# Shinzef/BlenderRayTracer

Measured on AMD Instinct MI355X. Metric: Msamples/s (pixels×spp/s) at 1/2/4/8 MI355X; % HBM roofline; RMS vs JS ref, higher is better.
Workload: dtype f64; 1 GPU; config3_rtow_1920x1080_512spp; scene=rtow.json, width=1920, height=1080, spp=512, max_depth=5, primitives=486, accel=auto, parallelism=1 GPU

## Files before the change

### __graft_entry__.py

```python
import os
import sys

ROOT = os.path.dirname(os.path.abspath(__file__))
if ROOT not in sys.path:
    sys.path.insert(0, ROOT)


def build() -> None:
    from blenderraytracer_amd import build as b
    b.build_lib(force=True)
    b.build_cli(force=True)
    b.build_napi(force=True)
    from oracle import binding
    binding.build()
    sys.path.insert(0, os.path.join(ROOT, "tests"))
    import hostcheck_binding
    hostcheck_binding.build()
    hostcheck_binding.lib(("RT_HOST_COUNTERS=1",))
    counting = ("RT_HOST_COUNTERS=1", "RT_TRI_FILTER=1")
    hostcheck_binding.lib(counting)
    hostcheck_binding.lib(counting + ("RT_TRI_EXIT=0",))
    hostcheck_binding.lib(("RT_HOST_COUNTERS=1", "RT_TRI_EXIT=0"))
    import texcheck_binding
    texcheck_binding.build()
    import lightcheck_binding
    lightcheck_binding.build()
    import guidedcheck_binding
    guidedcheck_binding.build()
    import neecheck_binding
    for mutation in (0, 1, 2):
        neecheck_binding.build(mutation)
    import filterxcheck_binding
    filterxcheck_binding.build()
    import errcheck_binding
    errcheck_binding.build()
    import vguidedcheck_binding
    vguidedcheck_binding.build()
    import blenderraytracer_amd
    from blenderraytracer_amd import capi
    capi.load_library()


def smoke() -> None:
    import numpy as np

    from blenderraytracer_amd import capi
    from blenderraytracer_amd.renderer import GpuRayTracer
    from blenderraytracer_amd.scene import load_scene_json
    from oracle import binding

    rt = GpuRayTracer(64, 48, seed=7, device=0, precision=capi.RT_PREC_F64)
    assert rt.load_from_json(load_scene_json("sample_scene.json"))
    rt.update_render_settings({"maxBounces": 4, "samples": 4})
    r = rt.render(want=("mean", "segments"))
    o = binding.render(rt.packed(), rt.settings())
    assert np.array_equal(r["segments"], o["segments"]), "segment counts differ from the oracle"
    err = np.max(np.abs(r["mean"] - o["mean"]))
    assert err <= 1e-12, f"GPU vs oracle max abs diff {err}"
    assert np.array_equal(r["rgba8"], o["rgba8"])
    print(f"smoke ok: 64x48x4spp sample_scene, {rt.last_stats.kernel_ms:.3f} ms kernel, max|diff| {err:.1e}")
    rt.close()
    rt = GpuRayTracer(48, 27, seed=7, device=0, precision=capi.RT_PREC_F64)
    assert rt.load_from_json(load_scene_json("rtow.json"))
    rt.update_render_settings({"maxBounces": 5, "samples": 4})
    lib = capi.load_library()
    assert lib.rt_scene_walk(rt.scene_handle(), capi.RT_PREC_F64, capi.RT_ACCEL_AUTO) == 2, "RTOW should walk the grid"
    r = rt.render(want=("mean", "segments"))
    o = binding.render(rt.packed(), rt.settings())
    assert np.array_equal(r["segments"], o["segments"]), "RTOW segment counts differ from the oracle"
    err = np.max(np.abs(r["mean"] - o["mean"]))
    assert err <= 1e-12, f"RTOW GPU vs oracle max abs diff {err}"
    assert np.array_equal(r["rgba8"], o["rgba8"])
    print(f"smoke ok: 48x27x4spp RTOW (grid walk), max|diff| {err:.1e}")
    rt.close()


if __name__ == "__main__":
    build()
    if len(sys.argv) > 1 and sys.argv[1] == "smoke":
        smoke()
```

### blenderraytracer_amd/build.py

```python
import hashlib
import json
import os
import shutil
import subprocess
import sys

HERE = os.path.dirname(os.path.abspath(__file__))
CSRC = os.path.join(HERE, "csrc")
LIBDIR = os.path.join(HERE, "lib")
REPO = os.path.dirname(HERE)
ARCH = os.environ.get("RT_OFFLOAD_ARCH", "gfx950")
HIPCC = os.environ.get("HIPCC", shutil.which("hipcc") or "/opt/rocm/bin/hipcc")

SOURCES = ["pt_trace.hip", "pt_onewave.hip", "pt_guided.hip", "pt_error.hip", "rt_capi.cpp", "scene_json.cpp"]
SOURCE_FLAGS = {"pt_onewave.hip": ["-mllvm", "-amdgpu-use-amdgpu-trackers=1"]}
HIP_FLAGS = ["-O3", "-std=c++17", f"--offload-arch={ARCH}", "-ffp-contract=off", "-fPIC",
             "-mllvm", "-structurizecfg-skip-uniform-regions=1",
             "-Wall", "-Wno-unused-function", "-I", os.path.join(REPO, "include")]


def _run(cmd):
    print(" ".join(cmd), flush=True)
    subprocess.check_call(cmd)

# ... 14 lines not shown
            if os.path.isfile(p):
                h.update(f.encode())
                with open(p, "rb") as fh:
                    h.update(fh.read())
    return h.hexdigest()[:16]


def _git(*args):
    try:
        return subprocess.run(["git", "-C", REPO, *args], capture_output=True, text=True, timeout=10).stdout.strip()
    except Exception:
        return ""


def write_build_info():
    info = {"commit": _git("rev-parse", "--short", "HEAD") or None,
            "sources_modified": bool(_git("status", "--porcelain", "--", CSRC, os.path.join(REPO, "include"),
                                          os.path.abspath(__file__))),
            "source_digest": source_digest()}
    with open(os.path.join(LIBDIR, "build_info.json"), "w") as f:
        json.dump(info, f)
    return info


def read_build_info():
    try:
        with open(os.path.join(LIBDIR, "build_info.json")) as f:
            return json.load(f)
    except (OSError, ValueError):
        return None


def build_lib(force=False):
    os.makedirs(LIBDIR, exist_ok=True)
    target = os.path.join(LIBDIR, "librt_hip.so")
    deps = [os.path.join(CSRC, f) for f in os.listdir(CSRC)] + [os.path.join(REPO, "include", f) for f in os.listdir(os.path.join(REPO, "include"))]
    if not force and not _stale(target, deps):
        return target
    objs, procs = [], []
    for src in SOURCES:
        obj = os.path.join(LIBDIR, os.path.splitext(src)[0] + ".o")
        cmd = [HIPCC, *HIP_FLAGS, *SOURCE_FLAGS.get(src, []), "-c", os.path.join(CSRC, src), "-o", obj]
        print(" ".join(cmd), flush=True)
        procs.append((cmd, subprocess.Popen(cmd)))
        objs.append(obj)
    failed = [cmd for cmd, p in procs if p.wait() != 0]
    if failed:
        raise subprocess.CalledProcessError(1, failed[0])
    _run([HIPCC, "-shared", f"--offload-arch={ARCH}", "-o", target, *objs])
    write_build_info()
    return target


def build_napi(force=False):
    node_inc = os.environ.get("NODE_INCLUDE", "/usr/include/node")
    if not os.path.exists(os.path.join(node_inc, "node_api.h")):
        print("node_api.h not found: skipping the N-API addon")
        return None
    target = os.path.join(LIBDIR, "rt_napi.node")
    src = os.path.join(CSRC, "napi_addon.cpp")
    if not os.path.exists(src):
        return None
    if not force and not _stale(target, [src, os.path.join(REPO, "include", "rt_hip.h"), os.path.join(LIBDIR, "librt_hip.so")]):
        return target
    _run(["g++", "-O2", "-std=c++17", "-fPIC", "-shared", "-I", node_inc, "-I", os.path.join(REPO, "include"),
          src, "-o", target, "-L", LIBDIR, "-lrt_hip", "-Wl,-rpath,$ORIGIN"])
    return target


def build_cli(force=False):
    target = os.path.join(LIBDIR, "rt_render_cli")
    src = os.path.join(CSRC, "rt_cli.cpp")
    deps = [src, os.path.join(LIBDIR, "librt_hip.so")] + [os.path.join(REPO, "include", f)
                                                          for f in os.listdir(os.path.join(REPO, "include"))]
    if not force and not _stale(target, deps):
        return target
    _run(["g++", "-O2", "-std=c++17", "-Wall", "-I", os.path.join(REPO, "include"), src, "-o", target,
          "-L", LIBDIR, "-lrt_hip", "-Wl,-rpath,$ORIGIN", "-Wl,-rpath-link,/opt/rocm/lib"])
    return target


def main(argv=None):
    argv = sys.argv[1:] if argv is None else argv
    force = "--force" in argv
    print(build_lib(force))
    print(build_cli(force))
    if "--napi" in argv:
        print(build_napi(force))


if __name__ == "__main__":
    main()
```

### blenderraytracer_amd/csrc/kernel_select.h

```cpp
#pragma once
#include <algorithm>
#include <cstdlib>
#include <cstring>
#include <type_traits>

#include "pt_core.h"

namespace rt {

#ifndef RT_MIN_WAVES_PER_SIMD
#define RT_MIN_WAVES_PER_SIMD 6
#endif
#ifndef RT_BVH_WAVES_PER_SIMD
#define RT_BVH_WAVES_PER_SIMD 4
#endif
#ifndef RT_BVH_WAVES_F32
#define RT_BVH_WAVES_F32 5
#endif

#ifndef RT_SPHERES_WAVES_PER_SIMD
#define RT_SPHERES_WAVES_PER_SIMD 5
#endif
#ifndef RT_SPHERES_WAVES_F32
#define RT_SPHERES_WAVES_F32 6
// ... 10 lines not shown
#define RT_GRID_WAVES_PER_SIMD 5
#endif
#ifndef RT_GRID_WAVES_F32
#define RT_GRID_WAVES_F32 6
#endif

template <class R, int ACC>
constexpr int waves_per_simd() {
    if constexpr (ACC == ACC_GRID || ACC == ACC_GRID_LDS || ACC == ACC_GRID_LDS_LEAN)
        return sizeof(R) == 8 ? RT_GRID_WAVES_PER_SIMD : RT_GRID_WAVES_F32;
    if constexpr (ACC == ACC_BVH_SPHERES) return sizeof(R) == 8 ? RT_SPHERES_WAVES_PER_SIMD : RT_SPHERES_WAVES_F32;
    if constexpr (ACC == ACC_BVH_SPHERES_LDS) return sizeof(R) == 8 ? RT_LDS_OCC_F64 : RT_LDS_OCC_F32;
    if constexpr (ACC == ACC_BVH_TRI_LDS) return sizeof(R) == 8 ? RT_BVH_WAVES_PER_SIMD : RT_BVH_WAVES_F32;
    return walk_of<ACC>() >= ACC_BVH ? (sizeof(R) == 8 ? RT_BVH_WAVES_PER_SIMD : RT_BVH_WAVES_F32) : RT_MIN_WAVES_PER_SIMD;
}

#ifndef RT_LDS_WAVES_F64
#define RT_LDS_WAVES_F64 8
#endif
#ifndef RT_LDS_WAVES_F32
#define RT_LDS_WAVES_F32 12
#endif
#ifndef RT_GRID_LDS_WAVES_F64
#define RT_GRID_LDS_WAVES_F64 4
#endif
#ifndef RT_GRID_LDS_WAVES_F32
#define RT_GRID_LDS_WAVES_F32 12
#endif
#ifndef RT_TRI_LDS_WAVES_F64
#define RT_TRI_LDS_WAVES_F64 16
#endif
#ifndef RT_TRI_LDS_WAVES_F32
#define RT_TRI_LDS_WAVES_F32 4
#endif
template <class R, int ACC = ACC_BVH_SPHERES_LDS>
constexpr int lds_waves() {
    if constexpr (ACC == ACC_GRID_LDS || ACC == ACC_GRID_LDS_LEAN) return sizeof(R) == 8 ? RT_GRID_LDS_WAVES_F64 : RT_GRID_LDS_WAVES_F32;
    if constexpr (ACC == ACC_BVH_TRI_LDS) return sizeof(R) == 8 ? RT_TRI_LDS_WAVES_F64 : RT_TRI_LDS_WAVES_F32;
    return sizeof(R) == 8 ? RT_LDS_WAVES_F64 : RT_LDS_WAVES_F32;
}

struct WideLds {
    int n, entries;
    RT_HD int boxes() const { return 0; }
    RT_HD int kids() const { return 48 * n; }
    RT_HD int stacks() const { return 56 * n; }
    RT_HD size_t bytes(int waves) const { return (size_t)56 * n + (size_t)waves * entries * 64 * 4; }
};
template <class R, int ACC>
constexpr long long lds_budget(int fewer_workgroups = 0) {
    return 160 * 1024 / (4 * waves_per_simd<R, ACC>() / lds_waves<R, ACC>() - fewer_workgroups);
}
template <class R, int ACC>
constexpr long long lds_fixed_bytes() { return (long long)lds_waves<R, ACC>() * 3 * 64 * 8 + 256; }

#ifndef RT_LDS_NODES
#define RT_LDS_NODES 1
#endif
#ifndef RT_LDS_GRID
#define RT_LDS_GRID 1
#endif
#ifndef RT_MAT_LDS
#define RT_MAT_LDS 0
#endif
#ifndef RT_LDS_TRI
#define RT_LDS_TRI 0
#endif
#ifndef RT_LEAN
#define RT_LEAN 1
#endif
constexpr int kWalkTree = -2;
inline int parse_bvh_walk(const char* e) {
    return e && !strncmp(e, "skip", 4) ? ACC_BVH : e && !strncmp(e, "two", 3) ? ACC_BVH_STACK
         : e && !strncmp(e, "grid", 4) ? ACC_GRID : e && !strncmp(e, "tree", 4) ? kWalkTree : ACC_BVH_SPHERES;
}
struct SelectKnobs {
    int bvh_walk = ACC_BVH_SPHERES;
    int lean = RT_LEAN;
    int lds_grid = RT_LDS_GRID;
    int lds_nodes = RT_LDS_NODES;
    int lds_tri = RT_LDS_TRI;
    int tri_lds_nodes = RT_TRI_TOP_NODES;
};
inline int env_int(const char* name, int def) {
    const char* e = getenv(name);
    return e ? atoi(e) : def;
}
inline SelectKnobs knobs_from_env() {
    SelectKnobs k;
    k.bvh_walk = parse_bvh_walk(getenv("RT_BVH_WALK"));
    k.lean = env_int("RT_LEAN", RT_LEAN);
    k.lds_grid = env_int("RT_LDS_GRID", RT_LDS_GRID);
    k.lds_nodes = env_int("RT_LDS_NODES", RT_LDS_NODES);
    k.lds_tri = env_int("RT_LDS_TRI", RT_LDS_TRI);
    k.tri_lds_nodes = std::max(0, std::min(env_int("RT_TRI_LDS_NODES", RT_TRI_TOP_NODES), RT_TRI_TOP_NODES));
    return k;
}

struct SceneFacts {
    int num_lights, num_tex, num_tri_nodes, num_tri_wide, num_sphere_wide, num_grid_cells, use_grid, num_planes,
        num_boxes, background, cam_ortho, stack_entries, num_mats;
    size_t grid_lds_bytes;
    int num_emitters;
};
template <class R>
SceneFacts scene_facts(const SceneView<R>& sc) {
    return SceneFacts{sc.num_lights, sc.num_tex, sc.num_tri_nodes, sc.num_tri_wide, sc.num_sphere_wide, sc.num_grid_cells,
                      sc.use_grid, sc.num_planes, sc.num_boxes, sc.background, sc.cam_ortho, sc.stack_entries,
                      sc.num_mats, grid_lds_bytes(sc), sc.num_emitters};
}

constexpr int kAccelCount = ACC_BVH_STACK_NEE + 1;
constexpr bool lds_form(int acc) {
    return acc == ACC_BVH_SPHERES_LDS || acc == ACC_GRID_LDS || acc == ACC_GRID_LDS_LEAN || acc == ACC_BVH_TRI_LDS;
}
constexpr int plain_of(int acc) {
    return acc == ACC_GRID_LDS_LEAN ? ACC_GRID_LDS : acc == ACC_BVH_STACK_LEAN ? ACC_BVH_STACK
         : acc == ACC_BRUTE_LEAN ? ACC_BRUTE : acc;
}
constexpr int walk_report(int acc) {
    return acc == ACC_BRUTE || acc == ACC_BRUTE_LEAN || acc == ACC_BRUTE_TEX || acc == ACC_BRUTE_LIT || acc == ACC_BRUTE_NEE ? 0
         : acc == ACC_GRID || acc == ACC_GRID_LDS || acc == ACC_GRID_LDS_LEAN ? 2 : 1;
}

struct KernelChoice {
    Accel acc;
    bool lds;
    size_t lds_bytes;
    int tri_lds_nodes;
};

template <int A = 0, class F>
auto with_acc(int acc, F&& f) -> decltype(f(std::integral_constant<int, 0>{})) {
    if constexpr (A + 1 == kAccelCount) return f(std::integral_constant<int, A>{});
    else return acc == A ? f(std::integral_constant<int, A>{}) : with_acc<A + 1>(acc, f);
}

template <class R>
KernelChoice select_kernel(const SceneFacts& s, int aa_mode, bool bvh, bool pool, const SelectKnobs& k) {
    const auto one_wave = [](Accel acc) { return KernelChoice{acc, false, 0, 0}; };
    if (s.num_emitters > 0) return one_wave(bvh ? ACC_BVH_STACK_NEE : ACC_BRUTE_NEE);
    if (s.num_lights > 0) return one_wave(bvh ? ACC_BVH_STACK_LIT : ACC_BRUTE_LIT);
    if (s.num_tex > 0) return one_wave(bvh ? ACC_BVH_STACK_TEX : ACC_BRUTE_TEX);
    const auto lean = [&](int feat) {
        if (k.lean == 0 || (k.lean == 2 && feat != 0)) return false;
        return (s.num_planes == 0 || (feat & F_PLANES)) && (s.num_boxes == 0 || (feat & F_BOXES)) &&
               (s.num_tri_nodes == 0 || (feat & F_TRIS)) && s.background == 0 && !s.cam_ortho && aa_mode == 0;
    };
    Accel walk = ACC_BRUTE;
    if (bvh && s.num_tri_nodes > 0) walk = k.bvh_walk == ACC_BVH ? ACC_BVH : ACC_BVH_STACK;
    else if (bvh && s.num_grid_cells > 0 && (k.bvh_walk == ACC_GRID || (k.bvh_walk == ACC_BVH_SPHERES && s.use_grid)))
        walk = ACC_GRID;
    else if (bvh) walk = k.bvh_walk == ACC_BVH || k.bvh_walk == ACC_BVH_STACK ? (Accel)k.bvh_walk : ACC_BVH_SPHERES;
    if (!pool) return one_wave(walk);
    const int entries = std::min(s.stack_entries, RT_BVH_STACK);
    if (walk == ACC_BRUTE && lean(feat_of<ACC_BRUTE_LEAN>())) return one_wave(ACC_BRUTE_LEAN);
    if (walk == ACC_GRID && k.lds_grid >= 1) {
        const size_t b = ((s.grid_lds_bytes + 15) & ~(size_t)15) + (RT_MAT_LDS ? sizeof(MatRec<R>) * (size_t)s.num_mats : 0);
        if ((long long)b + lds_fixed_bytes<R, ACC_GRID_LDS>() <= lds_budget<R, ACC_GRID_LDS>(RT_MAT_LDS ? 1 : 0))
            return KernelChoice{lean(feat_of<ACC_GRID_LDS_LEAN>()) ? ACC_GRID_LDS_LEAN : ACC_GRID_LDS, true, b, 0};
    }
    if (walk == ACC_BVH_SPHERES && k.lds_nodes >= (sizeof(R) == 8 ? 2 : 1) && s.num_sphere_wide > 0) {
        constexpr int W = lds_waves<R, ACC_BVH_SPHERES_LDS>();
        const size_t b = WideLds{s.num_sphere_wide, entries}.bytes(W);
        if ((long long)b + lds_fixed_bytes<R, ACC_BVH_SPHERES_LDS>() <= lds_budget<R, ACC_BVH_SPHERES_LDS>())
            return KernelChoice{ACC_BVH_SPHERES_LDS, true, b, 0};
    }
    if (walk == ACC_BVH_STACK) {
        if (k.lds_tri >= (sizeof(R) == 8 ? 1 : 2) && s.num_tri_wide > 0) {
            constexpr int W = lds_waves<R, ACC_BVH_TRI_LDS>();
            const long long fixed = (long long)W * entries * 64 * 4 + lds_fixed_bytes<R, ACC_BVH_TRI_LDS>();
            const long long n = std::min<long long>({(long long)s.num_tri_wide, (long long)k.tri_lds_nodes,
                                                     (lds_budget<R, ACC_BVH_TRI_LDS>() - fixed) / 56});
            if (n >= 64) return KernelChoice{ACC_BVH_TRI_LDS, true, WideLds{(int)n, entries}.bytes(W), (int)n};
        }
        if (lean(feat_of<ACC_BVH_STACK_LEAN>())) return one_wave(ACC_BVH_STACK_LEAN);
    }
    return one_wave(walk);
}

}
```

### blenderraytracer_amd/csrc/pt_core.h

```cpp
#pragma once
#include <hip/hip_runtime.h>
#include <math.h>
#include <stdint.h>
#include <string.h>
#include "js_math.h"

#define RT_HD __host__ __device__ __forceinline__
#ifndef RT_COLD_BG
#define RT_COLD_BG 1
#endif
#if RT_COLD_BG && defined(__HIP_DEVICE_COMPILE__)
#define RT_COLD __attribute__((noinline))
#else
#define RT_COLD
#endif
#define RT_COLD_HD __host__ __device__ RT_COLD

namespace rt {

template <class R> RT_HD R js_pow(R x, R y) {
    if constexpr (sizeof(R) == 8) return jsm::pow(x, y);
    else return pow(x, y);
}
template <class R> RT_HD R js_exp(R x) {
// ... 1234 lines not shown
    if ((e = fabs(p.y - b.mny)) < best) { best = e; n = mk<R>(0, -1, 0); }
    if ((e = fabs(p.y - b.mxy)) < best) { best = e; n = mk<R>(0, 1, 0); }
    if ((e = fabs(p.z - b.mnz)) < best) { best = e; n = mk<R>(0, 0, -1); }
    if ((e = fabs(p.z - b.mxz)) < best) { best = e; n = mk<R>(0, 0, 1); }
    return n;
}

template <class R, int FEAT = F_ALL>
RT_HD Hit<R> hit_record(const SceneView<R>& sc, V3<R> o, V3<R> d, const Closest<R>& c) {
    Hit<R> h;
    h.p = o + d * c.t;
    h.mat = c.mat;
    if ((FEAT & (F_PLANES | F_BOXES | F_TRIS)) == 0 || c.kind == HIT_SPHERE) {
        const SphereRec<R> s = sc.spheres[c.idx];
#if RT_DIV_RCP
        set_face(h, d, vdiv_rcp(h.p - mk(s.cx, s.cy, s.cz), sc.sphere_r[c.idx], sc.sphere_inv_r[c.idx]));
#else
        set_face(h, d, vdiv(h.p - mk(s.cx, s.cy, s.cz), sc.sphere_r[c.idx]));
#endif
    } else if ((FEAT & F_PLANES) != 0 && c.kind == HIT_PLANE) {
        const PlaneRec<R> p = sc.planes[c.idx];
        set_face(h, d, mk(p.nx, p.ny, p.nz));
    } else if ((FEAT & F_BOXES) != 0 && c.kind == HIT_BOX) {
        const BoxRec<R> b = sc.boxes[c.idx];
        const R eps = (R)1e-6;
        V3<R> n;
        if (fabs(h.p.x - b.mnx) < eps) n = mk<R>(-1, 0, 0);
        else if (fabs(h.p.x - b.mxx) < eps) n = mk<R>(1, 0, 0);
        else if (fabs(h.p.y - b.mny) < eps) n = mk<R>(0, -1, 0);
        else if (fabs(h.p.y - b.mxy) < eps) n = mk<R>(0, 1, 0);
        else if (fabs(h.p.z - b.mnz) < eps) n = mk<R>(0, 0, -1);
        else if (sizeof(R) == 8 || fabs(h.p.z - b.mxz) < eps) n = mk<R>(0, 0, 1);
        else n = box_nearest_face(h.p, b);
        set_face(h, d, n);
    } else {
        const TriRec<R> tr = sc.tris[c.idx];
        set_face(h, d, mk(tr.nx, tr.ny, tr.nz));
    }
    return h;
}

template <class R>
RT_HD V3<R> random_in_unit_sphere(Rng<R>& g) {
    int64_t x, y, z;
    do {
        RT_HCOUNT(HC_SPHERE_DRAW_ROUNDS, 1);
        x = (int64_t)g.next_u24() - (1 << 23);
        y = (int64_t)g.next_u24() - (1 << 23);
        z = (int64_t)g.next_u24() - (1 << 23);
    } while (x * x + y * y + z * z >= ((int64_t)1 << 46));
    return mk((R)x * (R)0x1p-23, (R)y * (R)0x1p-23, (R)z * (R)0x1p-23);
}

template <class R>
RT_HD V3<R> random_in_unit_disk(Rng<R>& g) {
    int64_t x, y;
    do {
        RT_HCOUNT(HC_DISK_DRAW_ROUNDS, 1);
        x = (int64_t)g.next_u24() - (1 << 23);
        y = (int64_t)g.next_u24() - (1 << 23);
    } while (x * x + y * y >= ((int64_t)1 << 46));
    return mk<R>((R)x * (R)0x1p-23, (R)y * (R)0x1p-23, 0);
}

template <class R> RT_HD R fade(R t) { return t * t * t * (t * (t * (R)6 - (R)15) + (R)10); }
template <class R> RT_HD R lerp(R t, R a, R b) { return a + t * (b - a); }
template <class R> RT_HD R grad(int hash, R x, R y, R z) {
    int h = hash & 15;
    R u = h < 8 ? x : y;
    R v = h < 4 ? y : (h == 12 || h == 14) ? x : z;
    return ((h & 1) == 0 ? u : -u) + ((h & 2) == 0 ? v : -v);
}
template <class R>
__host__ __device__ R perlin(const int* p, R x, R y, R z) {
    R fx0 = floor(x), fy0 = floor(y), fz0 = floor(z);
    int X = ((int)(long long)fx0) & 255, Y = ((int)(long long)fy0) & 255, Z = ((int)(long long)fz0) & 255;
    R fx = x - fx0, fy = y - fy0, fz = z - fz0;
    R u = fade(fx), v = fade(fy), w = fade(fz);
    int A = p[X] + Y, AA = p[A] + Z, AB = p[A + 1] + Z;
    int B = p[X + 1] + Y, BA = p[B] + Z, BB = p[B + 1] + Z;
    return lerp(w,
                lerp(v, lerp(u, grad(p[AA], fx, fy, fz), grad(p[BA], fx - (R)1, fy, fz)),
                     lerp(u, grad(p[AB], fx, fy - (R)1, fz), grad(p[BB], fx - (R)1, fy - (R)1, fz))),
                lerp(v, lerp(u, grad(p[AA + 1], fx, fy, fz - (R)1), grad(p[BA + 1], fx - (R)1, fy, fz - (R)1)),
                     lerp(u, grad(p[AB + 1], fx, fy - (R)1, fz - (R)1), grad(p[BB + 1], fx - (R)1, fy - (R)1, fz - (R)1))));
}


template <class R>
__host__ __device__ RT_COLD V3<R> background_hdri(const SceneView<R>& sc, V3<R> d) {
    const R I = sc.sky_intensity;
    V3<R> dir = normalize(d);
    V3<R> sun = normalize(mk<R>(-0.3, 0.6, -0.5));
    R sd = js_max<R>(0, dot(dir, sun));
    R mask = sd > ((R)1 - (R)0.04) ? (R)1 : (R)0;
    V3<R> sun_c = mk<R>(1.0, 0.95, 0.8) * (mask * (R)20);
    R corona = js_max<R>(0, (sd - ((R)1 - (R)0.2)) / (R)0.2);
    V3<R> cor_c = mk<R>(1.0, 0.8, 0.6) * (js_pow<R>(corona, (R)2) * (R)3);
    R y = dir.y;
    V3<R> sky_c = mk<R>(0.3, 0.5, 0.8) * (js_max<R>(0, y * (R)0.5 + (R)0.5) * (R)2);
    V3<R> gnd_c = mk<R>(0.2, 0.15, 0.1) * js_max<R>(0, -y * (R)0.3);
    V3<R> sc_c = mk<R>(0.8, 0.9, 1.0) * (js_pow<R>(js_max<R>(0, (R)1 - fabs(y)), (R)2) * (R)0.3);
    return ((((sky_c + gnd_c) + sc_c) + sun_c) + cor_c) * I;
}

template <class R>
// ... 150 lines not shown
```

### blenderraytracer_amd/csrc/pt_path.h

```cpp
#pragma once
#include <type_traits>

#include "pt_core.h"

namespace rt {

struct ImageParams {
    int width, height;
    int x0, y0, cw, ch;
    int samples;
    int s_begin, s_end;
    int max_depth;
    int aa_mode;
    uint32_t seedm;
    int pool_chunk;
    int batch_samples, batch_chunks;
    int batch_ways;
    int bands, band_chunks;
};

template <class R> struct AaUv { R u, v; };
template <class R>
RT_COLD_HD AaUv<R> stochastic_uv(uint32_t key, int i, int j, int width, int height) {
    Rng<R> g{key, 0};
// ... 186 lines not shown
    const int N = sc.num_emitters;
    if (N <= 0) return none;
    Rng<R> ge{lowbias32(key ^ lowbias32((uint32_t)bounce + 0x4E454531u)), 0};
    const EmitterDraw<R> s = sample_emitter(ev, N, h.p, ge);
    if (!s.ok) return none;
    const R cs = dot(h.n, s.om);
    if (!(cs > (R)0)) return none;
    const EmitterRec<R>& er = ev->recs[s.e];
    R te;
    if (!emitter_candidate(er, h.p, s.om, te)) return none;
    if (occluded<R, ACC>(sc, h.p, s.om, te, w, stk)) return none;
    const R pb = cs / (R)3.141592653589793;
    const R f = pb / (s.pO / (R)N + pb);
    return mk((att.x * er.le[0]) * f, (att.y * er.le[1]) * f, (att.z * er.le[2]) * f);
}

template <class R>
RT_HD bool emitter_hit_pdf(const SceneView<R>& sc, const Closest<R>& c, V3<R> o, V3<R> d, R& pO) {
    const EmitterView<R>* ev = emitter_view(sc);
    if (c.kind == HIT_SPHERE) {
        if (!ev->sphere_listed[c.idx]) return false;
        const SphereRec<R> s = sc.spheres[c.idx];
        const V3<R> w = mk(s.cx, s.cy, s.cz) - o;
        const R D2 = dot(w, w);
        if (!(D2 > s.r2)) return false;
        pO = cone_pdf(sphere_cone_omc(s.r2, D2));
        return true;
    }
    if (c.kind != HIT_TRI) return false;
    const R area = ev->tri_area[c.idx];
    if (!(area > (R)0)) return false;
    const TriRec<R> tr = sc.tris[c.idx];
    const R dd = dot(d, d);
    pO = tri_pdf((c.t * c.t) * dd, fabs(dot(mk(tr.nx, tr.ny, tr.nz), d)) / sqrt(dd), area);
    return true;
}
template <class R>
RT_HD R emission_weight(const SceneView<R>& sc, const Closest<R>& c, V3<R> o, V3<R> d, R pb) {
    if (!(pb > (R)0) || RT_NEE_MUTATION == 1) return (R)1;
    R pO;
    if (!emitter_hit_pdf(sc, c, o, d, pO)) return (R)1;
    return pb / (pb + (RT_NEE_MUTATION == 2 ? pO : pO / (R)sc.num_emitters));
}

template <class R> struct LightCtx { V3<R> dsum; Work* w; BvhStack stk; };
template <class R> struct NeeCtx : LightCtx<R> {
    R pb;
    int max_depth;
    RT_HD NeeCtx(V3<R> d, Work* w, BvhStack s) : LightCtx<R>{d, w, s}, pb((R)0), max_depth(0) {}
};
struct NoLightCtx { template <class... A> RT_HD NoLightCtx(A&&...) {} };
template <class R, bool LIT, bool NEE = false>
using LightState = std::conditional_t<NEE, NeeCtx<R>, std::conditional_t<LIT, LightCtx<R>, NoLightCtx>>;
template <class R, int FEAT = F_ALL, int ACC = ACC_BRUTE>
RT_HD bool shade_segment(const SceneView<R>& sc, const Closest<R>& c, V3<R>& o, V3<R>& d, V3<R>& T, int& depth,
                         Rng<R>& g, V3<R>& L, const MatRec<R>* mats = nullptr, LightCtx<R>* lc = nullptr) {
    bool done = true;
    L = mk<R>(0, 0, 0);
    const bool hit = c.kind != HIT_NONE;
    Hit<R> h{};
    MatRec<R> m{};
    V3<R> p = mk<R>(0, 0, 0);
    if (hit) {
        h = hit_record<R, FEAT>(sc, o, d, c);
        m = mats ? mats[h.mat] : sc.mats[h.mat];
        if (m.type <= 1) p = random_in_unit_sphere(g);
    }
    const V3<R> unit = normalize(hit && m.type == 0 ? p : d);
    if (hit) {
        if (m.type == 3) {
            RT_HCOUNT(HC_EMISSIVE, 1);
            L = mk(T.x * m.c[0], T.y * m.c[1], T.z * m.c[2]);
            if constexpr ((FEAT & F_NEE) != 0) {
                const R wgt = emission_weight<R>(sc, c, o, d, static_cast<NeeCtx<R>*>(lc)->pb);
                if (wgt != (R)1) L = L * wgt;
            }
        } else {
            V3<R> nd, att;
            if (scatter<R, (FEAT & F_TRIS) != 0 && (FEAT & F_ALL) != F_ALL>(m, h, unit, p, g, nd, att)) {
                if constexpr ((FEAT & F_TEX) != 0) {
                    if (m.type <= 1) {
                        const TexView<R>* tv = tex_view(sc);
                        const int tex = tv->mat_tex[h.mat];
                        if (tex >= 0) att = texture_value<R>(tv, tex, h.p);
                    }
                }
                if constexpr ((FEAT & F_LIGHT) != 0) {
                    if (m.type == 0) {
                        const V3<R> dl = direct_light<R, ACC>(sc, h, att, *lc->w, lc->stk);
                        lc->dsum = lc->dsum + mk(T.x * dl.x, T.y * dl.y, T.z * dl.z);
                    }
                }
                if constexpr ((FEAT & F_NEE) != 0) {
                    NeeCtx<R>* nc = static_cast<NeeCtx<R>*>(lc);
                    nc->pb = (R)0;
                    if (m.type == 0) {
                        if (depth > 1) {
                            const V3<R> el = emitter_light<R, ACC>(sc, h, att, g.key, nc->max_depth - depth, *nc->w, nc->stk);
                            nc->dsum = nc->dsum + mk(T.x * el.x, T.y * el.y, T.z * el.z);
                        }
                        nc->pb = dot(h.n, nd) / (sqrt(dot(nd, nd)) * (R)3.141592653589793);
                    }
                }
                T = mk(T.x * att.x, T.y * att.y, T.z * att.z);
                o = h.p;
                d = nd;
                done = --depth <= 0;
            }
        }
    } else {
        RT_HCOUNT(HC_MISS, 1);
        const V3<R> bg = background<R, FEAT>(sc, d, unit);
        L = mk(T.x * bg.x, T.y * bg.y, T.z * bg.z);
    }
    return done;
}

#ifndef RT_REC_DEPTH
#define RT_REC_DEPTH 16
#endif
// ... 178 lines not shown
```

### blenderraytracer_amd/csrc/pt_trace.hip

```cpp
#include <algorithm>
#include <atomic>
#include <chrono>
#include <cmath>
#include <cstdlib>
#include <cstring>
#include <mutex>
#include <thread>
#include <type_traits>
#include <vector>

#include "pt_launch.h"
#include "pt_error.h"
#include "kernel_select.h"
#include "pool_order.h"
#include "queue_slots.h"

namespace rt {

template <class R>
struct TraceArgs {
    SceneView<R> sc;
    ImageParams im;
    Counters c;
};
// ... 251 lines not shown
                __hip_atomic_fetch_add(&acc[m], (double)L.x, __ATOMIC_RELAXED, __HIP_MEMORY_SCOPE_WORKGROUP);
                __hip_atomic_fetch_add(&acc[64 + m], (double)L.y, __ATOMIC_RELAXED, __HIP_MEMORY_SCOPE_WORKGROUP);
                __hip_atomic_fetch_add(&acc[128 + m], (double)L.z, __ATOMIC_RELAXED, __HIP_MEMORY_SCOPE_WORKGROUP);
            }
        }
        const uint64_t t2 = RT_TICK();
        const uint64_t need = __ballot(waiting);
        if (need && (__popcll(need) >= defer_k || __ballot(!waiting) == 0)) {
            if (waiting) {
                const uint32_t k = next + __builtin_amdgcn_mbcnt_hi((uint32_t)(need >> 32),
                                                                    __builtin_amdgcn_mbcnt_lo((uint32_t)need, 0));
                live = k < total;
                if (live) begin_item(k);
                waiting = false;
            }
            next += (uint32_t)__popcll(need);
        }
        if (RT_PROFILE) res.cyc[2] += RT_TICK() - t2;
    }
    __syncthreads();
    if (lane < nv) {
        if (part) {
            double* p = part + ((size_t)item * 3) * 64 + lane;
            if (args.c.batch_count) {
                store_through(p, acc[lane]);
                store_through(p + 64, acc[64 + lane]);
                store_through(p + 128, acc[128 + lane]);
            } else {
                p[0] = acc[lane];
                p[64] = acc[64 + lane];
                p[128] = acc[128 + lane];
            }
        } else {
            const size_t qq = (size_t)(tl.y0 + lane / vw) * im.cw + (tl.x0 + lane % vw);
            args.c.sum[3 * qq] += acc[lane];
            args.c.sum[3 * qq + 1] += acc[64 + lane];
            args.c.sum[3 * qq + 2] += acc[128 + lane];
        }
    }
    if (args.c.batch_count) {
        if (im.bands) {
            const int bb = band_of_tile(im, tile);
            item_done(args.c, bb, band_items(im, bb), 1, lane);
        } else {
            item_done(args.c, cr.b, (uint32_t)(im.batch_chunks * tiles), im.batch_ways, lane);
        }
    }
    add_totals<ACC>(args.c, res, lane);
}

template <class R, bool COUNT, int ACC>
__device__ __forceinline__ void pool_item(const TraceArgs<R>& args, double* __restrict__ part, const int tiles,
                                          const int chunk, const unsigned pos, double* acc, BvhStack stk,
                                          PixelResult& res, const int lane, const MatRec<R>* lmats = nullptr) {
    const ImageParams& im = args.im;
    const SceneView<R>& sc = args.sc;
    const unsigned item = item_at(im, pos, tiles);
    const int tile = item % tiles;
    const ChunkRange cr = chunk_range(im, (int)(item / tiles), chunk);
    const Tile tl = tile_of(im, tile);
    const int vw = tl.vw, nv = tl.nv;
    const int sb = cr.sb, se = cr.se;
    const uint32_t total = (uint32_t)nv * (uint32_t)max(0, se - sb);
    int i = 0, j = 0, s = 0, depth = 0;
    uint32_t m = 0, pkey = 0, isegs = 0;
    size_t q = 0;
    Rng<R> g;
    V3<R> o, d, T;
    auto begin_item = [&](const uint32_t k) {
        uint32_t sr, mx, my;
        if (nv == 64) { m = k & 63; sr = k >> 6; }
        else { sr = k / (uint32_t)nv; m = k - sr * (uint32_t)nv; }
        if (RT_TILE_SHIFT && sizeof(R) == 8 && ACC == ACC_GRID_LDS_LEAN && nv == 64) { mx = m & 7; my = m >> 3; }
        else { mx = m % (uint32_t)vw; my = m / (uint32_t)vw; }
        const int px = tl.x0 + (int)mx, py = tl.y0 + (int)my;
        const int row = im.y0 + py;
        i = im.x0 + px;
        j = im.height - 1 - row;
        pkey = pixel_key(im.seedm, (uint32_t)row * (uint32_t)im.width + (uint32_t)i);
        q = (size_t)py * im.cw + px;
        s = sb + (int)sr;
        T = mk<R>(1, 1, 1);
        depth = im.max_depth;
        isegs = 0;
        start_sample<R, sizeof(R) == 4 || (RT_CAM_RELOAD_LEAN64 != 0 && ACC == ACC_GRID_LDS_LEAN), feat_of<ACC>()>(sc, im, i, j, pkey, s, g, o, d);
    };
    uint32_t next = 64;
    const int defer_k = defer_regen(sc);
    bool live = (uint32_t)lane < total;
    if (live) begin_item((uint32_t)lane);
    bool waiting = false;
    int origin = -1;
    while (live) {
        const uint64_t t0 = RT_TICK();
        if (!waiting) {
            const Closest<R> c = closest_hit_acc<R, ACC>(sc, o, d, res.work, stk, false, origin);
            const uint64_t t1 = RT_TICK();
            if (RT_PROFILE) res.cyc[0] += t1 - t0;
            ++res.segments;
            ++isegs;
            V3<R> L;
            waiting = shade_segment<R, feat_of<ACC>()>(sc, c, o, d, T, depth, g, L, lmats);
            if constexpr (RT_ORIGIN_LEAVE && sizeof(R) == 8 && ACC == ACC_GRID_LDS_LEAN)
                origin = !waiting && c.kind == HIT_SPHERE ? c.idx : -1;
            if (RT_PROFILE) res.cyc[1] += RT_TICK() - t1;
            if (waiting) {
                if (COUNT) {
                    if (args.c.segs) atomicAdd(args.c.segs + q, isegs);
                    if (args.c.draws) atomicAdd(args.c.draws + q, g.k);
                }
                __hip_atomic_fetch_add(&acc[m], (double)L.x, __ATOMIC_RELAXED, __HIP_MEMORY_SCOPE_WORKGROUP);
                __hip_atomic_fetch_add(&acc[64 + m], (double)L.y, __ATOMIC_RELAXED, __HIP_MEMORY_SCOPE_WORKGROUP);
                __hip_atomic_fetch_add(&acc[128 + m], (double)L.z, __ATOMIC_RELAXED, __HIP_MEMORY_SCOPE_WORKGROUP);
            }
        }
        const uint64_t t2 = RT_TICK();
        const uint64_t need = __ballot(waiting);
        if (need && (__popcll(need) >= defer_k || __ballot(!waiting) == 0)) {
            if (waiting) {
                const uint32_t k = next + __builtin_amdgcn_mbcnt_hi((uint32_t)(need >> 32),
                                                                    __builtin_amdgcn_mbcnt_lo((uint32_t)need, 0));
                live = k < total;
                if (live) begin_item(k);
                waiting = false;
            }
            next += (uint32_t)__popcll(need);
        }
        if (RT_PROFILE) res.cyc[2] += RT_TICK() - t2;
    }
    __builtin_amdgcn_fence(__ATOMIC_SEQ_CST, "wavefront");
    __builtin_amdgcn_wave_barrier();
    if (lane < nv) {
        if (part) {
            double* p = part + ((size_t)item * 3) * 64 + lane;
            if (args.c.batch_count) {
                store_through(p, acc[lane]);
                store_through(p + 64, acc[64 + lane]);
                store_through(p + 128, acc[128 + lane]);
            } else {
                p[0] = acc[lane];
                p[64] = acc[64 + lane];
                p[128] = acc[128 + lane];
            }
        } else {
            const size_t qq = (size_t)(tl.y0 + lane / vw) * im.cw + (tl.x0 + lane % vw);
            args.c.sum[3 * qq] += acc[lane];
            args.c.sum[3 * qq + 1] += acc[64 + lane];
            args.c.sum[3 * qq + 2] += acc[128 + lane];
        }
    }
    if (args.c.batch_count) {
        if (im.bands) {
            const int bb = band_of_tile(im, tile);
            item_done(args.c, bb, band_items(im, bb), 1, lane);
        } else {
// ... 16 lines not shown
        const rt_u4* g = reinterpret_cast<const rt_u4*>(src + k);
        const rt_u4 q3 = g[3];
        box[3 * k] = g[0];
        box[3 * k + 1] = g[1];
        box[3 * k + 2] = g[2];
        kid[k] = rt_u2{q3.x, q3.y};
    }
}

template <class R, bool COUNT, int ACC>
__global__ __launch_bounds__((64 * lds_waves<R, ACC>()), (waves_per_simd<R, ACC>()))
void trace_pool_lds_kernel(const TraceArgs<R> args, double* __restrict__ part, const int tiles, const int chunk,
                           const int items, const int qi) {
    constexpr int W = lds_waves<R, ACC>();
    const SceneView<R>& sc = args.sc;
    extern __shared__ __attribute__((aligned(16))) unsigned char lds_dyn[];
    __shared__ double acc_all[W * 3 * 64];
    const int wave = threadIdx.x >> 6, lane = threadIdx.x & 63;
    BvhStack stk{nullptr, 0};
    if constexpr (ACC == ACC_GRID_LDS || ACC == ACC_GRID_LDS_LEAN) {
        rt_u4* grec = reinterpret_cast<rt_u4*>(lds_dyn);
        int* gcell = reinterpret_cast<int*>(lds_dyn + grid_lds_rec_bytes(sc));
        copy_grid_lds<R, grid_filter_x<R, ACC>()>(sc, grec, gcell, threadIdx.x, 64 * W);
        stk.gcell = gcell;
        stk.grec = grec;
    } else if constexpr (ACC == ACC_BVH_TRI_LDS) {
        const int n = sc.tri_lds_nodes, entries = min(sc.stack_entries, RT_BVH_STACK);
        rt_u4* box = reinterpret_cast<rt_u4*>(lds_dyn);
        rt_u2* kid = reinterpret_cast<rt_u2*>(lds_dyn + 48 * n);
        int* stacks = reinterpret_cast<int*>(lds_dyn + 56 * n);
        copy_wide_lds(sc.tri_wide, n, box, kid, threadIdx.x, 64 * W);
        stk = BvhStack{stacks + wave * entries * 64 + lane, 64, box, kid};
        stk.ntop = n;
    } else {
        const int n = sc.num_sphere_wide, entries = min(sc.stack_entries, RT_BVH_STACK);
        rt_u4* box = reinterpret_cast<rt_u4*>(lds_dyn);
        rt_u2* kid = reinterpret_cast<rt_u2*>(lds_dyn + 48 * n);
        int* stacks = reinterpret_cast<int*>(lds_dyn + 56 * n);
        copy_wide_lds(sc.sphere_wide, n, box, kid, threadIdx.x, 64 * W);
        stk = BvhStack{stacks + wave * entries * 64 + lane, 64, box, kid};
    }
    double* acc = acc_all + wave * 3 * 64;
    acc[lane] = 0;
    acc[64 + lane] = 0;
    acc[128 + lane] = 0;
    const MatRec<R>* lmats = nullptr;
#if RT_MAT_LDS
    if constexpr (ACC == ACC_GRID_LDS || ACC == ACC_GRID_LDS_LEAN) {
        MatRec<R>* mm = reinterpret_cast<MatRec<R>*>(lds_dyn + ((grid_lds_bytes(sc) + 15) & ~(size_t)15));
        for (int k = threadIdx.x; k < sc.num_mats; k += 64 * W) mm[k] = sc.mats[k];
        lmats = mm;
    }
#endif
    __syncthreads();
    uint32_t* queue = g_pool_queue + 2 * qi;
    PixelResult res{0, 0, {0, 0, 0}, {0, 0, 0}};
    for (;;) {
        uint32_t it = 0;
        if (lane == 0) it = __hip_atomic_fetch_add(queue, 1u, __ATOMIC_RELAXED, __HIP_MEMORY_SCOPE_AGENT);
        it = (uint32_t)__builtin_amdgcn_readfirstlane((int)it);
        if (it >= (uint32_t)items) break;
        pool_item<R, COUNT, ACC>(args, part, tiles, chunk, it, acc, stk, res, lane, lmats);
    }
    add_totals<ACC>(args.c, res, lane);
    if (lane == 0) {
        const uint32_t e = __hip_atomic_fetch_add(queue + 1, 1u, __ATOMIC_RELAXED, __HIP_MEMORY_SCOPE_AGENT);
        if (e == gridDim.x * W - 1) {
            __hip_atomic_store(queue, 0u, __ATOMIC_RELAXED, __HIP_MEMORY_SCOPE_AGENT);
            __hip_atomic_store(queue + 1, 0u, __ATOMIC_RELAXED, __HIP_MEMORY_SCOPE_AGENT);
        }
    }
}

template <class F> struct FirstParam;
template <class A0, class... As> struct FirstParam<void (*)(A0, As...)> { using type = A0; };
static_assert(std::is_same<FirstParam<decltype(&trace_pool_lds_kernel<float, false, ACC_GRID_LDS>)>::type,
                           TraceArgs<float>>::value &&
              std::is_same<FirstParam<decltype(&trace_pool_lds_kernel<float, true, ACC_BVH_SPHERES_LDS>)>::type,
                           TraceArgs<float>>::value &&
              std::is_same<FirstParam<decltype(&trace_pool_lds_kernel<double, false, ACC_GRID_LDS_LEAN>)>::type,
                           TraceArgs<double>>::value &&
              std::is_same<FirstParam<decltype(&trace_pool_kernel<double, false, ACC_BVH_STACK_LEAN, false>)>::type,
                           TraceArgs<double>>::value,
              "the camera and grid reloads need TraceArgs as the LDS pool kernel's first (by-value) argument");

__global__ __launch_bounds__(64) void reduce_kernel(const ImageParams im, double* __restrict__ sum,
                                                    const double* __restrict__ part, const int tiles,
                                                    const int chunks, const uint32_t* __restrict__ skip,
                                                    const int tile0 = 0) {
    const int tile = tile0 + (int)blockIdx.x, m = threadIdx.x;
    if (tile >= tiles || (skip && *skip)) return;
    const Tile t = tile_of(im, tile);
    if (m >= t.nv) return;
    const size_t q = (size_t)(t.y0 + m / t.vw) * im.cw + (t.x0 + m % t.vw);
    double a0 = sum[3 * q], a1 = sum[3 * q + 1], a2 = sum[3 * q + 2];
    const double* p = part + (size_t)tile * 3 * 64 + m;
    const size_t stride = (size_t)tiles * 3 * 64;
    for (int c = 0; c < chunks; ++c, p += stride) {
        a0 += p[0];
        a1 += p[64];
        a2 += p[128];
    }
    sum[3 * q] = a0; sum[3 * q + 1] = a1; sum[3 * q + 2] = a2;
}

__global__ __launch_bounds__(64) void reduce_gate_kernel(const ReduceGate g) {
    if (threadIdx.x != 0) return;
    const uint32_t a = __hip_atomic_load(const_cast<uint32_t*>(g.aborted), __ATOMIC_RELAXED, __HIP_MEMORY_SCOPE_SYSTEM);
    const uint32_t s = __hip_atomic_load(g.stop, __ATOMIC_RELAXED, __HIP_MEMORY_SCOPE_SYSTEM);
    const uint32_t f = g.complete ? __hip_atomic_load(g.complete, __ATOMIC_ACQUIRE, __HIP_MEMORY_SCOPE_SYSTEM) : 1u;
    const uint32_t skip = (a | s) || !f ? 1u : 0u;
    *g.skip = skip;
    if (skip) __hip_atomic_store(g.stop, 1u, __ATOMIC_RELAXED, __HIP_MEMORY_SCOPE_SYSTEM);
    else __hip_atomic_store(g.done, g.done_value, __ATOMIC_RELAXED, __HIP_MEMORY_SCOPE_SYSTEM);
}
// ... 653 lines not shown
    idx_out[r] = hit ? c.idx : -1;
    double* rec = rec_out + 6 * r;
    if (!hit) {
        for (int k = 0; k < 6; ++k) rec[k] = (double)NAN;
        front_out[r] = 0;
        mat_out[r] = -1;
        return;
    }
    const Hit<R> h = hit_record<R, F_ALL>(sc, o, d, c);
    rec[0] = (double)h.p.x; rec[1] = (double)h.p.y; rec[2] = (double)h.p.z;
    rec[3] = (double)h.n.x; rec[4] = (double)h.n.y; rec[5] = (double)h.n.z;
    front_out[r] = h.front ? 1 : 0;
    mat_out[r] = h.mat;
}

template <class R>
hipError_t launch_hit_records(const SceneView<R>& sc, bool bvh, const double* rays, size_t n, double* t, int* kind,
                              int* idx, double* rec, uint8_t* front, int* mat, hipStream_t stream) {
    if (n == 0) return hipSuccess;
    const KernelChoice k = choose_kernel(sc, 0, bvh, true);
    SceneView<R> v = sc;
    if (k.acc == ACC_BVH_TRI_LDS) v.tri_lds_nodes = k.tri_lds_nodes;
    with_acc(k.acc, [&](auto tag) {
        constexpr int ACC = walk_of<plain_of(decltype(tag)::value)>();
        const size_t lb = !lds_form(ACC) ? 0 : ACC == ACC_GRID_LDS ? k.lds_bytes
                        : WideLds{ACC == ACC_BVH_TRI_LDS ? v.tri_lds_nodes : v.num_sphere_wide,
                                  std::min(v.stack_entries, RT_BVH_STACK)}.bytes(1);
        hipLaunchKernelGGL((hit_records_kernel<R, ACC>), dim3((unsigned)((n + 63) / 64)), dim3(64), lb, stream,
                           v, rays, n, t, kind, idx, rec, front, mat);
    });
    return hipGetLastError();
}
template hipError_t launch_hit_records<double>(const SceneView<double>&, bool, const double*, size_t, double*, int*, int*,
                                               double*, uint8_t*, int*, hipStream_t);
template hipError_t launch_hit_records<float>(const SceneView<float>&, bool, const double*, size_t, double*, int*, int*,
                                              double*, uint8_t*, int*, hipStream_t);

template <class R, int FEAT, int ACC>
__global__ __launch_bounds__(64) void shade_segments_kernel(const SceneView<R> sc, const double* __restrict__ rays,
                                                            const uint32_t* __restrict__ keys, const int depth0,
                                                            const size_t n, double* __restrict__ out_f,
                                                            int* __restrict__ out_i) {
    __shared__ int stack[RT_BVH_STACK * 64];
    const BvhStack stk{stack + threadIdx.x, 64};
    const size_t r = (size_t)blockIdx.x * 64 + threadIdx.x;
    if (r >= n) return;
    const double* q = rays + 6 * r;
    V3<R> o = mk<R>((R)q[0], (R)q[1], (R)q[2]), d = mk<R>((R)q[3], (R)q[4], (R)q[5]);
    Rng<R> g{keys[2 * r], keys[2 * r + 1]};
    V3<R> T = mk<R>(1, 1, 1), L;
    int depth = depth0;
    Work w{0, 0, 0, 0, 0, 0};
    const Closest<R> c = closest_hit_acc<R, ACC>(sc, o, d, w, stk);
    const bool done = shade_segment<R, FEAT, ACC>(sc, c, o, d, T, depth, g, L);
    double* f = out_f + 12 * r;
    f[0] = (double)o.x; f[1] = (double)o.y; f[2] = (double)o.z;
    f[3] = (double)d.x; f[4] = (double)d.y; f[5] = (double)d.z;
    f[6] = (double)T.x; f[7] = (double)T.y; f[8] = (double)T.z;
    f[9] = (double)L.x; f[10] = (double)L.y; f[11] = (double)L.z;
    int* k = out_i + 4 * r;
    k[0] = done ? 1 : 0;
    k[1] = c.kind;
    k[2] = c.kind == HIT_NONE ? -1 : c.idx;
    k[3] = (int)g.k;
}

template <class R>
hipError_t launch_shade_segments(const SceneView<R>& sc, bool bvh, int variant, const double* rays, const uint32_t* keys,
                                 int depth, size_t n, double* out_f, int* out_i, hipStream_t stream) {
    if (n == 0) return hipSuccess;
    if (variant < 0 || variant >= kShadeVariants) return hipErrorInvalidValue;
    const dim3 grid((unsigned)((n + 63) / 64));
    auto go = [&](auto feat) {
        constexpr int FEAT = decltype(feat)::value;
        if (bvh) hipLaunchKernelGGL((shade_segments_kernel<R, FEAT, ACC_BVH_STACK>), grid, dim3(64), 0, stream, sc, rays, keys, depth, n, out_f, out_i);
        else hipLaunchKernelGGL((shade_segments_kernel<R, FEAT, ACC_BRUTE>), grid, dim3(64), 0, stream, sc, rays, keys, depth, n, out_f, out_i);
    };
    if (variant == 0) go(std::integral_constant<int, F_ALL>{});
    else if (variant == 1) go(std::integral_constant<int, feat_of<ACC_BVH_STACK_LEAN>()>{});
    else go(std::integral_constant<int, feat_of<ACC_GRID_LDS_LEAN>()>{});
    return hipGetLastError();
}
template hipError_t launch_shade_segments<double>(const SceneView<double>&, bool, int, const double*, const uint32_t*, int,
                                                  size_t, double*, int*, hipStream_t);
template hipError_t launch_shade_segments<float>(const SceneView<float>&, bool, int, const double*, const uint32_t*, int,
                                                 size_t, double*, int*, hipStream_t);

template <class R, bool RELOAD, int FEAT>
__global__ __launch_bounds__(64) void camera_rays_kernel(const SceneView<R> sc, const ImageParams im,
                                                         const int* __restrict__ pixels, const size_t n,
                                                         double* __restrict__ out, uint32_t* __restrict__ draws) {
    const size_t r = (size_t)blockIdx.x * 64 + threadIdx.x;
    if (r >= n) return;
    const int i = pixels[3 * r], j = pixels[3 * r + 1], s = pixels[3 * r + 2];
    const int row = im.height - 1 - j;
    const uint32_t pkey = pixel_key(im.seedm, (uint32_t)row * (uint32_t)im.width + (uint32_t)i);
    Rng<R> g;
    V3<R> o, d;
    start_sample<R, RELOAD, FEAT>(sc, im, i, j, pkey, s, g, o, d);
    double* f = out + 6 * r;
    f[0] = (double)o.x; f[1] = (double)o.y; f[2] = (double)o.z;
    f[3] = (double)d.x; f[4] = (double)d.y; f[5] = (double)d.z;
    draws[r] = g.k;
}

template <class R>
hipError_t launch_camera_rays(const SceneView<R>& sc, const ImageParams& im, int variant, const int* pixels, size_t n,
// ... 229 lines not shown
```

Before: 11360 Msamples/s.

## Share unit-sphere rejection sampling across wave lanes via LDS slots

Replaces per-lane rejection sampling for the random point in the unit sphere with a wave-cooperative scheme. Lanes that still need a sample publish their RNG stream to per-wave LDS slots, and every lane in the wave evaluates candidate rounds for those streams. An atomic min picks the earliest accepted round, so the result matches sequential sampling. The aim is to cut divergent retry loops in the f64 lean grid kernel, at the cost of extra LDS per wave, ballots, wave barriers and atomics, plus a stricter LDS budget check for choosing the lean kernel.

```diff
diff --git a/__graft_entry__.py b/__graft_entry__.py
--- a/__graft_entry__.py
+++ b/__graft_entry__.py
@@ -11,6 +11,7 @@
     b.build_lib(force=True)
     b.build_cli(force=True)
     b.build_napi(force=True)
+    b.build_variant("coop0", ["RT_COOP_SPHERE=0"], force=True)
     from oracle import binding
     binding.build()
     sys.path.insert(0, os.path.join(ROOT, "tests"))
@@ -32,6 +33,11 @@
         neecheck_binding.build(mutation)
     import filterxcheck_binding
     filterxcheck_binding.build()
+    import coopcheck_binding
+    coopcheck_binding.build()
+    sys.path.insert(0, os.path.join(ROOT, "scripts"))
+    import wave_census
+    wave_census.build()
     import errcheck_binding
     errcheck_binding.build()
     import vguidedcheck_binding
diff --git a/blenderraytracer_amd/build.py b/blenderraytracer_amd/build.py
--- a/blenderraytracer_amd/build.py
+++ b/blenderraytracer_amd/build.py
@@ -90,6 +90,19 @@
     return target
 
 
+def build_variant(name, defines, force=False):
+    base = build_lib(force=False)
+    target = os.path.join(LIBDIR, f"librt_hip_{name}.so")
+    if not force and not _stale(target, [base]):
+        return target
+    obj = os.path.join(LIBDIR, f"pt_trace_{name}.o")
+    _run([HIPCC, *HIP_FLAGS, *SOURCE_FLAGS.get("pt_trace.hip", []), *[f"-D{d}" for d in defines], "-c",
+          os.path.join(CSRC, "pt_trace.hip"), "-o", obj])
+    objs = [obj if src == "pt_trace.hip" else os.path.join(LIBDIR, os.path.splitext(src)[0] + ".o") for src in SOURCES]
+    _run([HIPCC, "-shared", f"--offload-arch={ARCH}", "-o", target, *objs])
+    return target
+
+
 def build_napi(force=False):
     node_inc = os.environ.get("NODE_INCLUDE", "/usr/include/node")
     if not os.path.exists(os.path.join(node_inc, "node_api.h")):
diff --git a/blenderraytracer_amd/csrc/kernel_select.h b/blenderraytracer_amd/csrc/kernel_select.h
--- a/blenderraytracer_amd/csrc/kernel_select.h
+++ b/blenderraytracer_amd/csrc/kernel_select.h
@@ -86,7 +86,11 @@
     return 160 * 1024 / (4 * waves_per_simd<R, ACC>() / lds_waves<R, ACC>() - fewer_workgroups);
 }
 template <class R, int ACC>
-constexpr long long lds_fixed_bytes() { return (long long)lds_waves<R, ACC>() * 3 * 64 * 8 + 256; }
+constexpr long long coop_lds_bytes() {
+    return RT_COOP_SPHERE && sizeof(R) == 8 && ACC == ACC_GRID_LDS_LEAN ? (long long)lds_waves<R, ACC>() * 64 * 16 : 0;
+}
+template <class R, int ACC>
+constexpr long long lds_fixed_bytes() { return (long long)lds_waves<R, ACC>() * 3 * 64 * 8 + 256 + coop_lds_bytes<R, ACC>(); }
 
 #ifndef RT_LDS_NODES
 #define RT_LDS_NODES 1
@@ -191,8 +195,10 @@
     if (walk == ACC_BRUTE && lean(feat_of<ACC_BRUTE_LEAN>())) return one_wave(ACC_BRUTE_LEAN);
     if (walk == ACC_GRID && k.lds_grid >= 1) {
         const size_t b = ((s.grid_lds_bytes + 15) & ~(size_t)15) + (RT_MAT_LDS ? sizeof(MatRec<R>) * (size_t)s.num_mats : 0);
-        if ((long long)b + lds_fixed_bytes<R, ACC_GRID_LDS>() <= lds_budget<R, ACC_GRID_LDS>(RT_MAT_LDS ? 1 : 0))
-            return KernelChoice{lean(feat_of<ACC_GRID_LDS_LEAN>()) ? ACC_GRID_LDS_LEAN : ACC_GRID_LDS, true, b, 0};
+        const long long budget = lds_budget<R, ACC_GRID_LDS>(RT_MAT_LDS ? 1 : 0);
+        if (lean(feat_of<ACC_GRID_LDS_LEAN>()) && (long long)b + lds_fixed_bytes<R, ACC_GRID_LDS_LEAN>() <= budget)
+            return KernelChoice{ACC_GRID_LDS_LEAN, true, b, 0};
+        if ((long long)b + lds_fixed_bytes<R, ACC_GRID_LDS>() <= budget) return KernelChoice{ACC_GRID_LDS, true, b, 0};
     }
     if (walk == ACC_BVH_SPHERES && k.lds_nodes >= (sizeof(R) == 8 ? 2 : 1) && s.num_sphere_wide > 0) {
         constexpr int W = lds_waves<R, ACC_BVH_SPHERES_LDS>();
diff --git a/blenderraytracer_amd/csrc/pt_core.h b/blenderraytracer_amd/csrc/pt_core.h
--- a/blenderraytracer_amd/csrc/pt_core.h
+++ b/blenderraytracer_amd/csrc/pt_core.h
@@ -1310,6 +1310,47 @@
     return mk((R)x * (R)0x1p-23, (R)y * (R)0x1p-23, (R)z * (R)0x1p-23);
 }
 
+#ifndef RT_COOP_SPHERE
+#define RT_COOP_SPHERE 1
+#endif
+RT_HD bool sphere_round(uint32_t key, uint32_t k, uint32_t& ux, uint32_t& uy, uint32_t& uz) {
+    Rng<double> g{key, k};
+    ux = g.next_u24(); uy = g.next_u24(); uz = g.next_u24();
+    const int64_t x = (int64_t)ux - (1 << 23), y = (int64_t)uy - (1 << 23), z = (int64_t)uz - (1 << 23);
+    return x * x + y * y + z * z < ((int64_t)1 << 46);
+}
+RT_HD float coop_rcp(uint32_t n) {
+#if defined(__HIP_DEVICE_COMPILE__)
+    return __builtin_amdgcn_rcpf((float)(int)(n & 0x7Fu));
+#else
+    return 1.0f / (float)(int)(n & 0x7Fu);
+#endif
+}
+struct CoopShare { uint32_t q, j; };
+RT_HD CoopShare coop_assign(uint32_t h, uint32_t n, float rn) {
+    const uint32_t j = (uint32_t)(int)(((float)(int)(h & 0x7Fu) + 0.5f) * rn) & 0x7Fu;
+    return CoopShare{h - j * (n & 0x7Fu), j};
+}
+RT_HD uint32_t coop_rounds(uint32_t rho, uint32_t H, uint32_t n, float rn) {
+    const CoopShare a = coop_assign(H, n, rn);
+    return a.j + (rho < a.q ? 1u : 0u);
+}
+constexpr unsigned long long kCoopNone = ~0ull;
+RT_HD unsigned long long coop_pack(uint32_t j, uint32_t ux, uint32_t uy) {
+    return ((unsigned long long)j << 48) | ((unsigned long long)ux << 24) | (unsigned long long)uy;
+}
+RT_HD bool coop_take(unsigned long long word, uint32_t c, uint32_t& k, uint32_t& ux, uint32_t& uy) {
+    const uint32_t best = (uint32_t)(word >> 48);
+    if (best < c) {
+        k += 3 * (best + 1);
+        ux = (uint32_t)(word >> 24) & 0xFFFFFFu;
+        uy = (uint32_t)word & 0xFFFFFFu;
+        return true;
+    }
+    k += 3 * c;
+    return false;
+}
+
 template <class R>
 RT_HD V3<R> random_in_unit_disk(Rng<R>& g) {
     int64_t x, y;
diff --git a/blenderraytracer_amd/csrc/pt_path.h b/blenderraytracer_amd/csrc/pt_path.h
--- a/blenderraytracer_amd/csrc/pt_path.h
+++ b/blenderraytracer_amd/csrc/pt_path.h
@@ -262,20 +262,78 @@
 struct NoLightCtx { template <class... A> RT_HD NoLightCtx(A&&...) {} };
 template <class R, bool LIT, bool NEE = false>
 using LightState = std::conditional_t<NEE, NeeCtx<R>, std::conditional_t<LIT, LightCtx<R>, NoLightCtx>>;
+constexpr int kCoopSlotBytes = 16;
+#if defined(__HIP_DEVICE_COMPILE__)
+__device__ __forceinline__ uint32_t coop_rank(uint64_t mask) {
+    return __builtin_amdgcn_mbcnt_hi((uint32_t)(mask >> 32), __builtin_amdgcn_mbcnt_lo((uint32_t)mask, 0));
+}
+template <class R>
+__device__ __forceinline__ V3<R> unit_sphere_point(Rng<R>& g, bool need, unsigned long long* slots) {
+    uint32_t ux = 1u << 23, uy = 1u << 23, uz = 1u << 23;
+    if (need) {
+        need = !sphere_round(g.key, g.k, ux, uy, uz);
+        g.k += 3;
+    }
+    uint64_t N = __ballot(need);
+    while (N) {
+        const uint64_t E = __ballot(true);
+        const uint32_t n = (uint32_t)__popcll(N), H = (uint32_t)__popcll(E);
+        const uint32_t rho = coop_rank(N);
+        const float rn = coop_rcp(n);
+        __builtin_amdgcn_fence(__ATOMIC_SEQ_CST, "wavefront");
+        __builtin_amdgcn_wave_barrier();
+        if (need) {
+            slots[2 * rho] = ((unsigned long long)g.k << 32) | g.key;
+            slots[2 * rho + 1] = kCoopNone;
+        }
+        __builtin_amdgcn_fence(__ATOMIC_SEQ_CST, "wavefront");
+        __builtin_amdgcn_wave_barrier();
+        const CoopShare a = coop_assign(coop_rank(E), n, rn);
+        const unsigned long long stream = slots[2 * a.q];
+        uint32_t hx, hy, hz;
+        if (sphere_round((uint32_t)stream, (uint32_t)(stream >> 32) + 3 * a.j, hx, hy, hz))
+            __hip_atomic_fetch_min(slots + 2 * a.q + 1, coop_pack(a.j, hx, hy), __ATOMIC_RELAXED, __HIP_MEMORY_SCOPE_WORKGROUP);
+        __builtin_amdgcn_fence(__ATOMIC_SEQ_CST, "wavefront");
+        __builtin_amdgcn_wave_barrier();
+        if (need && coop_take(slots[2 * rho + 1], coop_rounds(rho, H, n, rn), g.k, ux, uy)) {
+            Rng<R> gz{g.key, g.k - 1};
+            uz = gz.next_u24();
+            need = false;
+        }
+        N = __ballot(need);
+    }
+    return mk((R)((int)ux - (1 << 23)) * (R)0x1p-23, (R)((int)uy - (1 << 23)) * (R)0x1p-23, (R)((int)uz - (1 << 23)) * (R)0x1p-23);
+}
+#endif
+template <class R, int FEAT>
+constexpr bool coop_sphere() {
+#if RT_COOP_SPHERE && defined(__HIP_DEVICE_COMPILE__)
+    return sizeof(R) == 8 && FEAT == feat_of<ACC_GRID_LDS_LEAN>();
+#else
+    return false;
+#endif
+}
 template <class R, int FEAT = F_ALL, int ACC = ACC_BRUTE>
 RT_HD bool shade_segment(const SceneView<R>& sc, const Closest<R>& c, V3<R>& o, V3<R>& d, V3<R>& T, int& depth,
-                         Rng<R>& g, V3<R>& L, const MatRec<R>* mats = nullptr, LightCtx<R>* lc = nullptr) {
+                         Rng<R>& g, V3<R>& L, const MatRec<R>* mats = nullptr, LightCtx<R>* lc = nullptr,
+                         unsigned long long* coop = nullptr) {
     bool done = true;
     L = mk<R>(0, 0, 0);
     const bool hit = c.kind != HIT_NONE;
     Hit<R> h{};
     MatRec<R> m{};
     V3<R> p = mk<R>(0, 0, 0);
+    const bool shared = coop_sphere<R, FEAT>() && coop != nullptr;
     if (hit) {
         h = hit_record<R, FEAT>(sc, o, d, c);
         m = mats ? mats[h.mat] : sc.mats[h.mat];
-        if (m.type <= 1) p = random_in_unit_sphere(g);
-    }
+        if (!shared && m.type <= 1) p = random_in_unit_sphere(g);
+    }
+#if defined(__HIP_DEVICE_COMPILE__)
+    if constexpr (coop_sphere<R, FEAT>()) {
+        if (shared) p = unit_sphere_point(g, hit && m.type <= 1, coop);
+    }
+#endif
     const V3<R> unit = normalize(hit && m.type == 0 ? p : d);
     if (hit) {
         if (m.type == 3) {
diff --git a/blenderraytracer_amd/csrc/pt_trace.hip b/blenderraytracer_amd/csrc/pt_trace.hip
--- a/blenderraytracer_amd/csrc/pt_trace.hip
+++ b/blenderraytracer_amd/csrc/pt_trace.hip
@@ -327,7 +327,8 @@
 template <class R, bool COUNT, int ACC>
 __device__ __forceinline__ void pool_item(const TraceArgs<R>& args, double* __restrict__ part, const int tiles,
                                           const int chunk, const unsigned pos, double* acc, BvhStack stk,
-                                          PixelResult& res, const int lane, const MatRec<R>* lmats = nullptr) {
+                                          PixelResult& res, const int lane, const MatRec<R>* lmats = nullptr,
+                                          unsigned long long* coop = nullptr) {
     const ImageParams& im = args.im;
     const SceneView<R>& sc = args.sc;
     const unsigned item = item_at(im, pos, tiles);
@@ -375,7 +376,7 @@
             ++res.segments;
             ++isegs;
             V3<R> L;
-            waiting = shade_segment<R, feat_of<ACC>()>(sc, c, o, d, T, depth, g, L, lmats);
+            waiting = shade_segment<R, feat_of<ACC>()>(sc, c, o, d, T, depth, g, L, lmats, nullptr, coop);
             if constexpr (RT_ORIGIN_LEAVE && sizeof(R) == 8 && ACC == ACC_GRID_LDS_LEAN)
                 origin = !waiting && c.kind == HIT_SPHERE ? c.idx : -1;
             if (RT_PROFILE) res.cyc[1] += RT_TICK() - t1;
@@ -498,6 +499,11 @@
         lmats = mm;
     }
 #endif
+    unsigned long long* coop = nullptr;
+    if constexpr (coop_lds_bytes<R, ACC>() > 0) {
+        __shared__ unsigned long long coop_all[coop_lds_bytes<R, ACC>() / 8];
+        coop = coop_all + wave * (64 * kCoopSlotBytes / 8);
+    }
     __syncthreads();
     uint32_t* queue = g_pool_queue + 2 * qi;
     PixelResult res{0, 0, {0, 0, 0}, {0, 0, 0}};
@@ -506,7 +512,7 @@
         if (lane == 0) it = __hip_atomic_fetch_add(queue, 1u, __ATOMIC_RELAXED, __HIP_MEMORY_SCOPE_AGENT);
         it = (uint32_t)__builtin_amdgcn_readfirstlane((int)it);
         if (it >= (uint32_t)items) break;
-        pool_item<R, COUNT, ACC>(args, part, tiles, chunk, it, acc, stk, res, lane, lmats);
+        pool_item<R, COUNT, ACC>(args, part, tiles, chunk, it, acc, stk, res, lane, lmats, coop);
     }
     add_totals<ACC>(args.c, res, lane);
     if (lane == 0) {
@@ -1266,7 +1272,12 @@
     int depth = depth0;
     Work w{0, 0, 0, 0, 0, 0};
     const Closest<R> c = closest_hit_acc<R, ACC>(sc, o, d, w, stk);
-    const bool done = shade_segment<R, FEAT, ACC>(sc, c, o, d, T, depth, g, L);
+    unsigned long long* coop = nullptr;
+    if constexpr (coop_sphere<R, FEAT>()) {
+        __shared__ unsigned long long coop_slots[64 * kCoopSlotBytes / 8];
+        coop = coop_slots;
+    }
+    const bool done = shade_segment<R, FEAT, ACC>(sc, c, o, d, T, depth, g, L, nullptr, nullptr, coop);
     double* f = out_f + 12 * r;
     f[0] = (double)o.x; f[1] = (double)o.y; f[2] = (double)o.z;
     f[3] = (double)d.x; f[4] = (double)d.y; f[5] = (double)d.z;
```

Measured after the change: 11540 Msamples/s, median of 6. +1.6%, better.
